# openpsi-project/srl

Hardware: AMD Instinct MI355X
Metric: env-steps/sec through GAE+PPO update, 4096 envs x 128 steps (higher is better)
Workload: dtype f32 (contractions as bf16x3 / f16x2 piece products, float32 accumulate)

## Files before the change

srl_amd/csrc/h2conv.h:

```cpp
#pragma once
#include "h2gemm.h"

namespace srlh2 {

typedef float h2_f32x4 __attribute__((ext_vector_type(4)));

enum { H2C_F2 = 0, H2C_F3 = 1, H2C_D3 = 2, H2C_D2 = 3 };
enum { H2S_LINEAR = 0, H2S_PLANAR = 1, H2S_ROWS = 2, H2S_ROWSWZ = 3 };
enum { H2D_PLANAR = 0, H2D_ROWS = 1, H2D_F32_ROUTED = 2 };

template <int ID> struct H2Geo;

template <> struct H2Geo<H2C_F2> {
  static constexpr int CGW = 1;
  static constexpr int CB = 1, NCH = 64, NTAP = 16, GW = 10, OH = 9, OW = 9, NPIX_L = 400, G = 1, PLANE_E = 400;
  static constexpr int SRC = H2S_ROWSWZ, PAD = 0, SH = 20, SW = 20, SPIX = 400;
  static constexpr int DST = H2D_PLANAR, OPIX = 81, OCH = 64;
  static constexpr bool ZERO_BORDER = false;
  static constexpr bool DENSE = false;
  __host__ __device__ static constexpr int tap_u(int t) { return (((t >> 2) & 1) * 2 + (t & 1)) * 100 + (t >> 3) * 10 + ((t & 3) >> 1); }
  __host__ __device__ static constexpr int tap_k(int t) { return t; }
};
template <> struct H2Geo<H2C_F3> {
  static constexpr int CGW = 1;
  static constexpr int CB = 2, NCH = 64, NTAP = 9, GW = 9, OH = 7, OW = 7, NPIX_L = 81, G = 2, PLANE_E = 176;
  static constexpr int SRC = H2S_PLANAR, PAD = 0, SH = 9, SW = 9, SPIX = 81;
  static constexpr int DST = H2D_ROWS, OPIX = 49, OCH = 64;
  static constexpr bool ZERO_BORDER = false;
  static constexpr bool DENSE = false;
  __host__ __device__ static constexpr int tap_u(int t) { return (t / 3) * 9 + t % 3; }
  __host__ __device__ static constexpr int tap_k(int t) { return t; }
};
template <> struct H2Geo<H2C_D3> {
  static constexpr int CGW = 1;
  static constexpr int CB = 2, NCH = 64, NTAP = 9, GW = 11, OH = 9, OW = 9, NPIX_L = 121, G = 2, PLANE_E = 256;
  static constexpr int SRC = H2S_ROWS, PAD = 2, SH = 7, SW = 7, SPIX = 49;
  static constexpr int DST = H2D_PLANAR, OPIX = 81, OCH = 64;
  static constexpr bool ZERO_BORDER = true;
  static constexpr bool DENSE = true;
  __host__ __device__ static constexpr int tap_u(int t) { return (2 - t / 3) * 11 + (2 - t % 3); }
  __host__ __device__ static constexpr int tap_k(int t) { return t; }
};
template <> struct H2Geo<H2C_D2> {
  static constexpr int CGW = 2;
  static constexpr int CB = 2, NCH = 128, NTAP = 4, GW = 11, OH = 10, OW = 10, NPIX_L = 121, G = 2, PLANE_E = 256;
  static constexpr int SRC = H2S_PLANAR, PAD = 1, SH = 9, SW = 9, SPIX = 81;
  static constexpr int DST = H2D_F32_ROUTED, OPIX = 400, OCH = 32;
  static constexpr bool ZERO_BORDER = true;
  static constexpr bool DENSE = true;
  __host__ __device__ static constexpr int tap_u(int t) { return (1 - t / 2) * 11 + (1 - t % 2); }
  __host__ __device__ static constexpr int tap_k(int t) { return t; }
};

struct H2ConvArgs {
  const void* x;
  const void* w;
  const float* sx;
  const float* sw;
  int64_t n;
  const float* bias;
  int32_t act;
  void* out;
  float* out_scale;
  const float* bound_in;
  const float* bound_w;
  const float* bound_b;
  float* out_absmax;
  uint8_t* mask_out;
  const void* mask_in;
};

#ifdef __HIPCC__

template <int ID> constexpr int h2c_src_img_bytes() { return H2Geo<ID>::SPIX * H2Geo<ID>::CB * 128; }
template <int ID> constexpr int h2c_slot_bytes() { return H2Geo<ID>::CB * 8 * H2Geo<ID>::PLANE_E * 16; }

__device__ __forceinline__ uint32_t h2_xor32(uint32_t x, bool upper) {
#if __has_builtin(__builtin_amdgcn_permlane32_swap)
  typedef unsigned h2_u32x2 __attribute__((ext_vector_type(2)));
  const h2_u32x2 r = __builtin_amdgcn_permlane32_swap(x, x, false, false);
  return upper ? r[0] : r[1];
#else
  (void)upper;
  return (uint32_t)__shfl_xor((int)x, 32);
#endif
}

#ifndef SRL_H2C_SCHED
#define SRL_H2C_SCHED 1
#endif

template <int NKB> struct H2ActiveKb { int n; int kb[NKB]; };
template <int RM, int NTAP, int CB, int TPR> constexpr H2ActiveKb<NTAP * CB> h2_active_kbs() {
  H2ActiveKb<NTAP * CB> a{};
  for (int kb = 0; kb < NTAP * CB; ++kb)
    if ((RM >> ((kb / CB) / TPR)) & 1) a.kb[a.n++] = kb;
  return a;
}

template <int ID, int NSLOT>
__global__ __launch_bounds__(512, 2) void h2conv_kernel(H2ConvArgs a) {
  using GE = H2Geo<ID>;
  constexpr int CB = GE::CB, NKB = GE::NTAP * CB, NPL = CB * 8, PLANE_B = GE::PLANE_E * 16;
  constexpr int SLOT = NPL * PLANE_B;
  constexpr int NCG = GE::NCH / 16;
  constexpr int CGW = GE::CGW, NWG = NCG / CGW;
  constexpr int NPH = 8 / NWG;
  static_assert(NWG == 4 || NWG == 8, "");
  constexpr int NE = GE::DENSE ? GE::OH * GE::OW : (GE::OH - 1) * GE::GW + GE::OW;
  constexpr int NB_IMG = (NE + 15) / 16;
  constexpr int NBT = NB_IMG * GE::G;
  static_assert(NBT % NPH == 0 && NPH <= 2, "blocks split evenly over the (at most two) position halves");
  constexpr int NDMA = SLOT / 1024;
  constexpr int NDW = (NDMA + 7) / 8;
  static_assert(SLOT % 1024 == 0, "");
  constexpr int KROW = NKB * 128;
  constexpr int IMGB = h2c_src_img_bytes<ID>();
  constexpr bool ROUTED = GE::DST == H2D_F32_ROUTED;
  constexpr int OIMGB = GE::OPIX * GE::OCH * 4;
  constexpr int MIMGB = GE::OPIX * GE::OCH / 8;
  constexpr bool MASK_IN = ID == H2C_D3 || ID == H2C_D2, MASK_OUT = !MASK_IN;
  constexpr int MREG = MASK_IN ? (GE::G * MIMGB + 1023) / 1024 * 1024 : 0;
  constexpr int SLOTM = SLOT + MREG;
  constexpr int NDM = MREG / 1024;
  extern __shared__ __attribute__((aligned(1024))) uint8_t lds[];

  const int tid = threadIdx.x, lane = tid & 63;
  const int wid = __builtin_amdgcn_readfirstlane(tid >> 6);
  const int cg0 = (wid % NWG) * CGW, ph = wid / NWG;
  const int p = lane & 15, quad = lane >> 4;
  const bool up = quad >> 1;

  h2_f16x8 wf[CGW][NKB][2];
  {
#pragma unroll
    for (int c = 0; c < CGW; ++c) {
      const uint8_t* wr = static_cast<const uint8_t*>(a.w) + (size_t)((cg0 + c) * 16 + p) * KROW + quad * 32;
#pragma unroll
      for (int kb = 0; kb < NKB; ++kb) {
        wf[c][kb][0] = *reinterpret_cast<const h2_f16x8*>(wr + kb * 128);
        wf[c][kb][1] = *reinterpret_cast<const h2_f16x8*>(wr + kb * 128 + 16);
      }
    }
#pragma unroll
    for (int c = 0; c < CGW; ++c)
#pragma unroll
      for (int kb = 0; kb < NKB; ++kb) asm volatile("" : "+v"(wf[c][kb][0]), "+v"(wf[c][kb][1]));
  }
  const float inv = 1.f / (*a.sx * *a.sw);
  float oscale = 1.f;
  if (!ROUTED) {
    float bound = *a.bound_in * *a.bound_w;
    if (a.bound_b) bound += *a.bound_b;
    oscale = h2_scale_for(bound);
    if (blockIdx.x == 0 && tid == 0) *a.out_scale = oscale;
  }
  float bq[CGW][4];
#pragma unroll
  for (int c = 0; c < CGW; ++c) {
    bq[c][0] = bq[c][1] = bq[c][2] = bq[c][3] = 0.f;
    if (a.bias) {
      const float4 b4 = *reinterpret_cast<const float4*>(a.bias + (cg0 + c) * 16 + 4 * quad);
      bq[c][0] = b4.x; bq[c][1] = b4.y; bq[c][2] = b4.z; bq[c][3] = b4.w;
    }
  }
  const float lo = a.act == 1 ? 0.f : -3.0e38f;

  if (GE::ZERO_BORDER) {
    for (int i = tid; i < NSLOT * SLOTM / 16; i += 512) reinterpret_cast<uint4*>(lds)[i] = make_uint4(0, 0, 0, 0);
    __syncthreads();
  }

  const h2_i32x4 rx = h2_rsrc(a.x);
  h2_i32x4 rmd = h2_rsrc(MASK_IN ? a.mask_in : a.x);
  rmd[2] = MASK_IN ? (int)(a.n * MIMGB) : 0;
  const uint32_t lds0 = (uint32_t)(uintptr_t)(__attribute__((address_space(3))) uint8_t*)lds;
  const long nbatch = (a.n + GE::G - 1) / GE::G;

  uint32_t dvoff[NDW];
  int dimg[NDW];
#pragma unroll
  for (int q = 0; q < NDW; ++q) {
    const int j = wid + 8 * q;
    const int nent = j * 64 + lane;
    if (GE::SRC == H2S_LINEAR) {
      dvoff[q] = (uint32_t)(nent * 16);
      dimg[q] = j < NDMA ? 0 : -1;
    } else if (GE::SRC == H2S_ROWSWZ) {
      const int P = nent >> 3, sl = nent & 7;
      dvoff[q] = (uint32_t)(P * 128 + 16 * (sl ^ (((P >> 1) & 1) | (((P >> 2) & 1) << 2))));
      dimg[q] = j < NDMA ? 0 : -1;
    } else {
      const int plane = nent / GE::PLANE_E, e = nent - plane * GE::PLANE_E;
      const int il = e / GE::NPIX_L, cell = e - il * GE::NPIX_L;
      const int gy = cell / GE::GW, gx = cell - gy * GE::GW;
      const int sy = gy - GE::PAD, sx = gx - GE::PAD;
      const bool ok = j < NDMA && il < GE::G && (unsigned)sy < (unsigned)GE::SH && (unsigned)sx < (unsigned)GE::SW;
      const int sp = sy * GE::SW + sx;
      if (GE::SRC == H2S_PLANAR) dvoff[q] = (uint32_t)(il * IMGB + plane * (GE::SPIX * 16) + sp * 16);
      else dvoff[q] = (uint32_t)((il * GE::SPIX + sp) * (CB * 128) + plane * 16);
      dimg[q] = ok ? il : -1;
      if (!ok) dvoff[q] = 0;
    }
  }
  auto issue = [&](long b, int s) {
    const long img0 = b * GE::G;
    const int left = (int)(a.n - img0 < GE::G ? a.n - img0 : GE::G);
    const uint32_t soff = __builtin_amdgcn_readfirstlane((uint32_t)(img0 * (long)IMGB));
#pragma unroll
    for (int q = 0; q < NDW; ++q) {
      const uint32_t ldsa = __builtin_amdgcn_readfirstlane(lds0 + s * SLOTM + (wid + 8 * q) * 1024);
      if (dimg[q] >= 0 && dimg[q] < left)
        asm volatile("s_mov_b32 m0, %0\n\ts_nop 4\n\tbuffer_load_dwordx4 %1, %2, %3 offen lds" ::"s"(ldsa), "v"(dvoff[q]), "s"(rx), "s"(soff) : "memory");
    }
    if (MASK_IN && wid < NDM) {
      const uint32_t ldsa = __builtin_amdgcn_readfirstlane(lds0 + s * SLOTM + SLOT + wid * 1024);
      const uint32_t msoff = __builtin_amdgcn_readfirstlane((uint32_t)(img0 * (long)MIMGB));
      const uint32_t mvoff = (uint32_t)(wid * 1024 + lane * 16);
      asm volatile("s_mov_b32 m0, %0\n\ts_nop 4\n\tbuffer_load_dwordx4 %1, %2, %3 offen lds" ::"s"(ldsa), "v"(mvoff), "s"(rmd), "s"(msoff) : "memory");
    }
  };

  uint32_t lane_out[CGW];
  uint32_t lane_mout[CGW];
  int mi_shift[CGW], mi_pix[CGW];
  int pix_step_y, pix_step_x;
#pragma unroll
  for (int c = 0; c < CGW; ++c) {
    const int cg = cg0 + c;
    const int g_out = 2 * (quad & 1) + (cg & 1), ocb = cg >> 1;
    if (ROUTED) {
      const int cls = cg >> 1, py = cls >> 1, px = cls & 1;
      lane_out[c] = (uint32_t)(((py * 20 + px) * GE::OCH + 16 * (cg & 1) + 4 * quad) * 4);
      lane_mout[c] = 0;
      mi_shift[c] = 16 * (cg & 1) + 4 * quad;
      mi_pix[c] = py * 20 + px;
    } else {
      lane_out[c] = GE::DST == H2D_PLANAR ? (uint32_t)((((ocb * 4 + g_out) * 2 + (up ? 1 : 0)) * GE::OPIX) * 16)
                                          : (uint32_t)(ocb * 128 + g_out * 32 + (up ? 16 : 0));
      lane_mout[c] = (uint32_t)(ocb * 4 + g_out);
      mi_shift[c] = 0;
      mi_pix[c] = 0;
    }
  }
  if (ROUTED) { pix_step_y = 40; pix_step_x = 2; }
  else { pix_step_y = GE::OW; pix_step_x = 1; }
  constexpr int PIXB = ROUTED ? GE::OCH * 4 : (GE::DST == H2D_PLANAR ? 16 : GE::OCH * 4);
  const uint32_t lane_base = GE::SRC == H2S_ROWSWZ ? (uint32_t)(p * 128 + quad * 32) : (uint32_t)(quad * 2 * PLANE_B + p * 16);
  int swz_d0[8], swz_d1[8];
  if (GE::SRC == H2S_ROWSWZ) {
    static_assert(GE::SRC != H2S_ROWSWZ || SLOTM % 128 == 0, "slot stride must keep address bits 4-6");
    const uint32_t a_ref = (uint32_t)(uintptr_t)(lds + lane_base);
#pragma unroll
    for (int u = 0; u < 8; ++u) {
      const int k = (p + u) & 7;
      const uint32_t x = (uint32_t)((((k >> 1) & 1) | (((k >> 2) & 1) << 2)) * 16);
      swz_d0[u] = u * 128 + (int)((a_ref ^ x) - a_ref);
      swz_d1[u] = u * 128 + (int)((a_ref ^ x ^ 16u) - a_ref);
    }
  }
  float amax = 0.f;

  struct Meta {
    uint32_t pixoff;
    bool ok;
    long img;
    uint32_t bits[CGW];
  };
  const __amdgpu_buffer_rsrc_t r_out = __builtin_amdgcn_make_buffer_rsrc(a.out, 0, (int)(a.n * OIMGB), 0x00020000);
  const __amdgpu_buffer_rsrc_t r_mo = __builtin_amdgcn_make_buffer_rsrc(MASK_OUT ? (void*)a.mask_out : a.out, 0, (int)(a.n * MIMGB), 0x00020000);
  constexpr uint32_t OOB = 0x80000000u;
  auto epilogue1 = [&](const h2_f32x4& acc, const Meta& m, const float (&bqc)[4], uint32_t lane_out_c, uint32_t lane_mout_c, uint32_t mbits) {
    float v[4];
    constexpr bool CLAMP = ID == H2C_F2 || ID == H2C_F3;
#pragma unroll
    for (int r = 0; r < 4; ++r) v[r] = CLAMP ? fmaxf(acc[r] * inv + bqc[r], lo) : acc[r] * inv + bqc[r];
    const bool ok = m.ok;
    const uint32_t img32 = (uint32_t)m.img;
    if (MASK_IN) {
#pragma unroll
      for (int r = 0; r < 4; ++r) v[r] = __uint_as_float(__float_as_uint(v[r]) & (uint32_t)__builtin_amdgcn_sbfe((int)mbits, r, 1));
    }
    {
      const float m3 = __builtin_fmaxf(__builtin_fmaxf(fabsf(v[0]), fabsf(v[1])), fabsf(v[2]));
      const float m5 = __builtin_fmaxf(__builtin_fmaxf(m3, fabsf(v[3])), amax);
      amax = m.ok ? m5 : amax;
    }
    const uint32_t ooff = ok ? m.pixoff * PIXB + lane_out_c : OOB;
    typedef uint32_t h2_u32x4 __attribute__((ext_vector_type(4)));
    if (ROUTED) {
      h2_u32x4 d = {__float_as_uint(v[0]), __float_as_uint(v[1]), __float_as_uint(v[2]), __float_as_uint(v[3])};
      __builtin_amdgcn_raw_buffer_store_b128(d, r_out, ooff + img32 * (uint32_t)OIMGB, 0, 0);
    } else {
      uint32_t h0a, h0b, h1a, h1b;
      h2_split_pair(v[0], v[1], oscale, h0a, h1a);
      h2_split_pair(v[2], v[3], oscale, h0b, h1b);
      h2_u32x4 chunk;
#if __has_builtin(__builtin_amdgcn_permlane32_swap)
      typedef unsigned h2_u32x2 __attribute__((ext_vector_type(2)));
      const h2_u32x2 sa = __builtin_amdgcn_permlane32_swap(h0a, h1a, false, false);
      const h2_u32x2 sb = __builtin_amdgcn_permlane32_swap(h0b, h1b, false, false);
      chunk[0] = sa[0]; chunk[1] = sb[0]; chunk[2] = sa[1]; chunk[3] = sb[1];
#else
      const uint32_t r0 = h2_xor32(up ? h0a : h1a, up), r1 = h2_xor32(up ? h0b : h1b, up);
      chunk[0] = up ? r0 : h0a; chunk[1] = up ? r1 : h0b; chunk[2] = up ? h1a : r0; chunk[3] = up ? h1b : r1;
#endif
      __builtin_amdgcn_raw_buffer_store_b128(chunk, r_out, ooff + img32 * (uint32_t)OIMGB, 0, 0);
      if (MASK_OUT) {
        uint32_t nib = (v[0] > 0.f ? 1u : 0u) | (v[1] > 0.f ? 2u : 0u) | (v[2] > 0.f ? 4u : 0u) | (v[3] > 0.f ? 8u : 0u);
#if __has_builtin(__builtin_amdgcn_permlane32_swap)
        const h2_u32x2 sn = __builtin_amdgcn_permlane32_swap(nib, nib, false, false);
        const uint32_t byte = sn[0] | (sn[1] << 4);
#else
        const uint32_t byte = nib | (h2_xor32(nib, up) << 4);
#endif
        const uint32_t moff = (ok && !up) ? m.pixoff * (GE::OCH / 8) + lane_mout_c : OOB;
        __builtin_amdgcn_raw_buffer_store_b8((unsigned char)byte, r_mo, moff + img32 * (uint32_t)MIMGB, 0, 0);
      }
    }
  };
  auto epilogue = [&](const h2_f32x4 (&accs)[CGW], const Meta& m) {
#pragma unroll
    for (int c = 0; c < CGW; ++c) epilogue1(accs[c], m, bq[c], lane_out[c], lane_mout[c], m.bits[c]);
  };

  constexpr int PD = CB == 1 ? 3 : (ID == H2C_D2 ? 1 : 2);
  const bool late = wid >= 4;
  auto block = [&](auto rows_c, const uint8_t* xb, h2_f32x4 (&pacc)[CGW], Meta& pm, const Meta& nm) {
    constexpr int TPR = ID == H2C_D3 ? 3 : (ID == H2C_D2 ? 2 : GE::NTAP);
    constexpr H2ActiveKb<NKB> AK = h2_active_kbs<decltype(rows_c)::value, GE::NTAP, CB, TPR>();
    h2_f32x4 acc[CGW];
#pragma unroll
    for (int c = 0; c < CGW; ++c) acc[c] = h2_f32x4{0.f, 0.f, 0.f, 0.f};
    h2_f16x8 xr[PD + 1][2];
    const uint8_t* tq0[8];
    const uint8_t* tq1[8];
    if (GE::SRC == H2S_ROWSWZ) {
#pragma unroll
      for (int u = 0; u < 8; ++u) {
        tq0[u] = xb + swz_d0[u];
        tq1[u] = xb + swz_d1[u];
      }
    }
    auto fetch = [&](int i) {
      const int kb = AK.kb[i];
      const int t = kb / CB, c = kb - t * CB;
      if (GE::SRC == H2S_ROWSWZ) {
        const int U = GE::tap_u(t), u8 = U & 7;
        xr[i % (PD + 1)][0] = *reinterpret_cast<const h2_f16x8*>(tq0[u8] + (U - u8) * 128);
        xr[i % (PD + 1)][1] = *reinterpret_cast<const h2_f16x8*>(tq1[u8] + (U - u8) * 128);
      } else {
        const int off = (c * 8) * PLANE_B + GE::tap_u(t) * 16;
        xr[i % (PD + 1)][0] = *reinterpret_cast<const h2_f16x8*>(xb + off);
        xr[i % (PD + 1)][1] = *reinterpret_cast<const h2_f16x8*>(xb + off + PLANE_B);
      }
    };
#pragma unroll
    for (int i = 0; i < PD; ++i) fetch(i);
#pragma unroll
    for (int i = 0; i < AK.n; ++i) {
      if (i + PD < AK.n) fetch(i + PD);
      if (i == 1 && !late) epilogue(pacc, pm);
      if (i == AK.n / 2 + 1 && late) epilogue(pacc, pm);
      const int kb = AK.kb[i];
      const int t = kb / CB, c = kb - t * CB;
      const int kw = GE::tap_k(t) * CB + c;
#pragma unroll
      for (int cc = 0; cc < CGW; ++cc) {
        acc[cc] = __builtin_amdgcn_mfma_f32_16x16x32_f16(wf[cc][kw][1], xr[i % (PD + 1)][0], acc[cc], 0, 0, 0);
        acc[cc] = __builtin_amdgcn_mfma_f32_16x16x32_f16(wf[cc][kw][0], xr[i % (PD + 1)][1], acc[cc], 0, 0, 0);
        acc[cc] = __builtin_amdgcn_mfma_f32_16x16x32_f16(wf[cc][kw][0], xr[i % (PD + 1)][0], acc[cc], 0, 0, 0);
      }
    }
#pragma unroll
    for (int c = 0; c < CGW; ++c) pacc[c] = acc[c];
    pm = nm;
  };

  h2_f32x4 pacc[CGW];
#pragma unroll
  for (int c = 0; c < CGW; ++c) pacc[c] = h2_f32x4{0.f, 0.f, 0.f, 0.f};
  Meta pm = {};
  pm.ok = false;
  auto compute = [&](auto phc_c, long b, int s) {
    constexpr int phc = decltype(phc_c)::value;
    const uint8_t* slot = lds + s * SLOTM + lane_base;
    const uint8_t* mreg = lds + s * SLOTM + SLOT;
#pragma unroll
    for (int jj = 0; jj < NBT / NPH; ++jj) {
      const int jb = phc * (NBT / NPH) + jj;
      const int il = jb / NB_IMG, bi = jb - il * NB_IMG;
      const int e = bi * 16 + p;
      constexpr int EW = GE::DENSE ? GE::OW : GE::GW;
      const int oy = (e * (65536 / EW + 1)) >> 16, ox = e - oy * EW;
      Meta nm;
      nm.img = b * GE::G + il;
      nm.ok = ox < GE::OW && oy < GE::OH && nm.img < a.n;
      nm.pixoff = (uint32_t)(oy * pix_step_y + ox * pix_step_x);
#pragma unroll
      for (int c = 0; c < CGW; ++c) {
        nm.bits[c] = 0u;
        if (MASK_IN) {
          const uint32_t po = nm.ok ? nm.pixoff : 0u;
          if (ID == H2C_D3) nm.bits[c] = (uint32_t)mreg[il * MIMGB + po * (GE::OCH / 8) + lane_mout[c]] >> (up ? 4 : 0);
          else nm.bits[c] = *reinterpret_cast<const uint32_t*>(mreg + il * MIMGB + (po + mi_pix[c]) * 4) >> mi_shift[c];
        }
      }
      const uint8_t* xb_ = slot + (il * GE::NPIX_L + bi * 16) * (GE::SRC == H2S_ROWSWZ ? 128 : 16) +
                           (GE::DENSE ? oy * ((GE::GW - GE::OW) * 16) : 0);
      if (ID == H2C_D3) {
        static_assert(ID != H2C_D3 || (NB_IMG == 6 && GE::GW == 11 && GE::OW == 9 && GE::NTAP == 9 && GE::SRC != H2S_ROWSWZ),
                      "row masks below are conv3's");
        if (bi == 0) block(std::integral_constant<int, 0b011>{}, xb_, pacc, pm, nm);
        else if (bi == 4) block(std::integral_constant<int, 0b110>{}, xb_, pacc, pm, nm);
        else if (bi == 5) block(std::integral_constant<int, 0b100>{}, xb_, pacc, pm, nm);
        else block(std::integral_constant<int, 0b111>{}, xb_, pacc, pm, nm);
      } else if (ID == H2C_D2) {
        static_assert(ID != H2C_D2 || (NB_IMG == 7 && GE::GW == 11 && GE::OW == 10 && GE::NTAP == 4), "row mask below is conv2's");
        if (bi == 6) block(std::integral_constant<int, 0b10>{}, xb_, pacc, pm, nm);
        else block(std::integral_constant<int, 0b11>{}, xb_, pacc, pm, nm);
      } else {
        block(std::integral_constant<int, (1 << 30) - 1>{}, xb_, pacc, pm, nm);
      }
    }
  };

  long b = blockIdx.x;
#pragma unroll
  for (int s = 0; s < NSLOT - 1; ++s)
    if (b + (long)s * gridDim.x < nbatch) issue(b + (long)s * gridDim.x, s);
  int s_cur = 0, s_nxt = NSLOT - 1;
  for (; b < nbatch; b += gridDim.x) {
    asm volatile("s_waitcnt vmcnt(0)\n\ts_waitcnt lgkmcnt(0)" ::: "memory");
    __builtin_amdgcn_s_barrier();
    const long bn = b + (long)(NSLOT - 1) * gridDim.x;
    if (bn < nbatch) issue(bn, s_nxt);
    if (ph == 0) compute(std::integral_constant<int, 0>{}, b, s_cur);
    else compute(std::integral_constant<int, NPH - 1>{}, b, s_cur);
    s_cur = s_cur + 1 == NSLOT ? 0 : s_cur + 1;
    s_nxt = s_nxt + 1 == NSLOT ? 0 : s_nxt + 1;
  }
  epilogue(pacc, pm);
  {
#pragma unroll
    for (int o = 32; o >= 1; o >>= 1) amax = fmaxf(amax, __shfl_xor(amax, o));
    if (lane == 0) {
      const float cur = __hip_atomic_load(a.out_absmax, __ATOMIC_RELAXED, __HIP_MEMORY_SCOPE_AGENT);
      if (amax > cur) atomicMax(reinterpret_cast<int*>(a.out_absmax), __float_as_int(amax));
    }
  }
}

template <int ID, int NSLOT = 2>
inline int h2conv_launch(hipStream_t st, const H2ConvArgs& a, int max_blocks = 256) {
  constexpr bool MASK_IN_L = ID == H2C_D3 || ID == H2C_D2;
  constexpr int SLOT = h2c_slot_bytes<ID>() + (MASK_IN_L ? (H2Geo<ID>::G * (H2Geo<ID>::OPIX * H2Geo<ID>::OCH / 8) + 1023) / 1024 * 1024 : 0);
  static_assert(NSLOT * SLOT <= 160 * 1024, "LDS");
  static bool attr_set = false;
  auto kern = h2conv_kernel<ID, NSLOT>;
  if (!attr_set) {
    (void)hipFuncSetAttribute(reinterpret_cast<const void*>(kern), hipFuncAttributeMaxDynamicSharedMemorySize, NSLOT * SLOT);
    attr_set = true;
  }
  const long nbatch = (a.n + H2Geo<ID>::G - 1) / H2Geo<ID>::G;
  if (nbatch <= 0) return 0;
  const long grid = nbatch < max_blocks ? nbatch : max_blocks;
  hipLaunchKernelGGL(kern, dim3((unsigned)grid), dim3(512), NSLOT * SLOT, st, a);
  return 0;
}

__host__ __device__ inline int h2_entry(int y, int x, int H, int W, int order) {
  return order == 2 ? ((y & 1) * 2 + (x & 1)) * ((H / 2) * (W / 2)) + (y >> 1) * (W / 2) + (x >> 1) : y * W + x;
}
static __global__ void h2_pack_planar_kernel(const float* __restrict__ src, int64_t n, int H, int W, int C, int order, const float* absmax,
                                      const float* scale_in, float* scale_out, uint8_t* __restrict__ dst) {
  const float scale = scale_in ? *scale_in : h2_scale_for(*absmax);
  if (scale_out && blockIdx.x == 0 && threadIdx.x == 0) *scale_out = scale;
  const int64_t ngrp = n * H * W * (C / 8);
  for (int64_t t = (int64_t)blockIdx.x * blockDim.x + threadIdx.x; t < ngrp; t += (int64_t)gridDim.x * blockDim.x) {
    const int gi = (int)(t % (C / 8));
    int64_t r = t / (C / 8);
    const int x = (int)(r % W); r /= W;
    const int y = (int)(r % H);
    const int64_t img = r / H;
    const int blk = gi >> 2, g = gi & 3;
    const float* s = src + ((img * H + y) * W + x) * C + blk * 32;
    float v[8];
#pragma unroll
    for (int j = 0; j < 8; ++j) v[j] = s[h2p_elem(g, j)];
    uint4 h0, h1;
    h2_split_pair(v[0], v[1], scale, h0.x, h1.x);
    h2_split_pair(v[2], v[3], scale, h0.y, h1.y);
    h2_split_pair(v[4], v[5], scale, h0.z, h1.z);
    h2_split_pair(v[6], v[7], scale, h0.w, h1.w);
    const int NP = H * W, e = h2_entry(y, x, H, W, order);
    uint8_t* d = dst + img * (int64_t)(NP * C * 4);
    *reinterpret_cast<uint4*>(d + ((int64_t)((blk * 4 + g) * 2 + 0) * NP + e) * 16) = h0;
    *reinterpret_cast<uint4*>(d + ((int64_t)((blk * 4 + g) * 2 + 1) * NP + e) * 16) = h1;
  }
}
static __global__ void h2_pack_pixrows_kernel(const float* __restrict__ src, int64_t n, int H, int W, int C, int order, const float* absmax,
                                       const float* scale_in, float* scale_out, uint8_t* __restrict__ dst) {
  const float scale = scale_in ? *scale_in : h2_scale_for(*absmax);
  if (scale_out && blockIdx.x == 0 && threadIdx.x == 0) *scale_out = scale;
  const int64_t ngrp = n * H * W * (C / 8);
  for (int64_t t = (int64_t)blockIdx.x * blockDim.x + threadIdx.x; t < ngrp; t += (int64_t)gridDim.x * blockDim.x) {
    const int gi = (int)(t % (C / 8));
    int64_t r = t / (C / 8);
    const int x = (int)(r % W); r /= W;
    const int y = (int)(r % H);
    const int64_t img = r / H;
    const int blk = gi >> 2, g = gi & 3;
    const float* s = src + ((img * H + y) * W + x) * C + blk * 32;
    float v[8];
#pragma unroll
    for (int j = 0; j < 8; ++j) v[j] = s[h2p_elem(g, j)];
    uint4 h0, h1;
    h2_split_pair(v[0], v[1], scale, h0.x, h1.x);
    h2_split_pair(v[2], v[3], scale, h0.y, h1.y);
    h2_split_pair(v[4], v[5], scale, h0.z, h1.z);
    h2_split_pair(v[6], v[7], scale, h0.w, h1.w);
    uint4* d = reinterpret_cast<uint4*>(dst + ((img * (int64_t)(H * W) + h2_entry(y, x, H, W, order)) * C + blk * 32) * 4 + g * 32);
    d[0] = h0;
    d[1] = h1;
  }
}
static __global__ void h2_unpack_planar_kernel(const uint8_t* __restrict__ src, int64_t n, int H, int W, int C, int order, const float* scale,
                                        float* __restrict__ dst) {
  const float inv = 1.f / *scale;
  const int64_t ngrp = n * H * W * (C / 8);
  for (int64_t t = (int64_t)blockIdx.x * blockDim.x + threadIdx.x; t < ngrp; t += (int64_t)gridDim.x * blockDim.x) {
    const int gi = (int)(t % (C / 8));
    int64_t r = t / (C / 8);
    const int x = (int)(r % W); r /= W;
    const int y = (int)(r % H);
    const int64_t img = r / H;
    const int blk = gi >> 2, g = gi & 3;
    const int NP = H * W, e = h2_entry(y, x, H, W, order);
    const uint8_t* d = src + img * (int64_t)(NP * C * 4);
    const _Float16* p0 = reinterpret_cast<const _Float16*>(d + ((int64_t)((blk * 4 + g) * 2 + 0) * NP + e) * 16);
    const _Float16* p1 = reinterpret_cast<const _Float16*>(d + ((int64_t)((blk * 4 + g) * 2 + 1) * NP + e) * 16);
    float* o = dst + ((img * H + y) * W + x) * C + blk * 32;
#pragma unroll
    for (int j = 0; j < 8; ++j) o[h2p_elem(g, j)] = ((float)p0[j] + (float)p1[j]) * inv;
  }
}

#endif

enum { H2W_C2 = 0, H2W_C3 = 1 };

template <int ID> struct H2WGeo;
template <> struct H2WGeo<H2W_C2> {
  static constexpr int CIN = 32, NTAP = 16, GW = 10, OH = 9, OW = 9, XPIX = 400, ZPIX = 81, ZW = 9;
  static constexpr bool X_ROWS = true, Z_ROWS = false;
  static constexpr int MC = 4, NN = 4;
  __host__ __device__ static constexpr int tap_u(int t) { return (((t >> 2) & 1) * 2 + (t & 1)) * 100 + (t >> 3) * 10 + ((t & 3) >> 1); }
};
template <> struct H2WGeo<H2W_C3> {
  static constexpr int CIN = 64, NTAP = 9, GW = 9, OH = 7, OW = 7, XPIX = 81, ZPIX = 49, ZW = 7;
  static constexpr bool X_ROWS = false, Z_ROWS = true;
  static constexpr int MC = 2, NN = 9;
  __host__ __device__ static constexpr int tap_u(int t) { return (t / 3) * 9 + t % 3; }
};

struct H2WgradArgs {
  const void* x;
  const void* dz;
  const float* sx;
  const float* sz;
  int64_t n;
  float* slabs;
};

#ifdef __HIPCC__

typedef short h2_s16x4 __attribute__((ext_vector_type(4)));

__host__ __device__ constexpr int h2w_plane_base(int idx, int plane) { return idx * plane + (idx >> 3) * 256 + (((idx >> 1) & 3) >= 2 ? 128 : 0); }

__device__ __forceinline__ h2_s16x4 h2_tr_read(const uint8_t* p) {
  typedef __attribute__((address_space(3))) h2_s16x4 lds_s16x4;
  return __builtin_amdgcn_ds_read_tr16_b64_v4i16((lds_s16x4*)p);
}

template <int ID, int NSLOT>
__global__ __launch_bounds__(512, 2) void h2wgrad_kernel(H2WgradArgs a) {
  using GE = H2WGeo<ID>;
  constexpr int CBX = GE::CIN / 32;
  constexpr int NE = (GE::OH - 1) * GE::GW + GE::OW;
  constexpr int NCHUNK = (NE + 31) / 32;
  constexpr int ZE = NCHUNK * 32;
  constexpr int ZPLANE = ZE * 16;
  constexpr int ZBYTES = 16 * ZPLANE + 512;
  constexpr int XE = GE::X_ROWS ? GE::XPIX : ((GE::XPIX + 15) / 16) * 16;
  constexpr int XPLANE = XE * 16;
  constexpr int XBYTES = GE::X_ROWS ? GE::XPIX * 128 : CBX * 8 * XPLANE + CBX * 256;
  constexpr int XB_AL = (XBYTES + 1023) / 1024 * 1024, ZB_AL = (ZBYTES + 1023) / 1024 * 1024;
  constexpr int SLOT = XB_AL + ZB_AL;
  constexpr int NDX = XB_AL / 1024, NDZ = ZB_AL / 1024, NDMA = NDX + NDZ, NDW = (NDMA + 7) / 8;
  constexpr int K = GE::NTAP * GE::CIN;
  constexpr int XIMGB = GE::XPIX * GE::CIN * 4, ZIMGB = GE::ZPIX * 64 * 4;
  static_assert(NSLOT * SLOT <= 160 * 1024, "LDS");
  extern __shared__ __attribute__((aligned(1024))) uint8_t lds[];

  const int tid = threadIdx.x, lane = tid & 63;
  const int wid = __builtin_amdgcn_readfirstlane(tid >> 6);
  const int o = lane >> 4, q = (lane >> 2) & 3, p = lane & 3;

  for (int i = tid; i < NSLOT * SLOT / 16; i += 512) reinterpret_cast<uint4*>(lds)[i] = make_uint4(0, 0, 0, 0);
  __syncthreads();

  const h2_i32x4 rx = h2_rsrc(a.x), rz = h2_rsrc(a.dz);
  const uint32_t lds0 = (uint32_t)(uintptr_t)(__attribute__((address_space(3))) uint8_t*)lds;
  int dvoff[NDW];
#pragma unroll
  for (int qd = 0; qd < NDW; ++qd) {
    const int j = wid + 8 * qd;
    int off = -1;
    if (j < NDX) {
      const int b = j * 1024 + lane * 16;
      if (GE::X_ROWS) {
        const int P = b >> 7, sl = (b >> 4) & 7;
        if (P < GE::XPIX) off = P * 128 + 16 * (sl ^ (((P >> 1) & 1) | (((P >> 2) & 1) << 2)));
      } else {
#pragma unroll
        for (int pl_i = 0; pl_i < CBX * 8; ++pl_i) {
          const int rel = b - h2w_plane_base(pl_i, XPLANE);
          if (rel >= 0 && rel < XPLANE && (rel >> 4) < GE::XPIX) off = pl_i * (GE::XPIX * 16) + (rel >> 4) * 16;
        }
      }
    } else if (j < NDMA) {
      const int b = (j - NDX) * 1024 + lane * 16;
#pragma unroll
      for (int pl_i = 0; pl_i < 16; ++pl_i) {
        const int rel = b - h2w_plane_base(pl_i, ZPLANE);
        if (rel >= 0 && rel < ZPLANE) {
          const int e = rel >> 4, oy = e / GE::GW, ox = e - oy * GE::GW;
          if (ox < GE::OW && oy < GE::OH) {
            const int zp = oy * GE::ZW + ox;
            off = GE::Z_ROWS ? zp * 256 + pl_i * 16 : pl_i * (GE::ZPIX * 16) + zp * 16;
          }
        }
      }
    }
    dvoff[qd] = off;
  }
  auto issue = [&](long img, int s) {
    const uint32_t sox = __builtin_amdgcn_readfirstlane((uint32_t)(img * (long)XIMGB));
    const uint32_t soz = __builtin_amdgcn_readfirstlane((uint32_t)(img * (long)ZIMGB));
#pragma unroll
    for (int qd = 0; qd < NDW; ++qd) {
      const int j = wid + 8 * qd;
      const uint32_t ldsa = __builtin_amdgcn_readfirstlane(lds0 + s * SLOT + j * 1024);
      if (dvoff[qd] >= 0) {
        if (j < NDX) asm volatile("s_mov_b32 m0, %0\n\ts_nop 4\n\tbuffer_load_dwordx4 %1, %2, %3 offen lds" ::"s"(ldsa), "v"(dvoff[qd]), "s"(rx), "s"(sox) : "memory");
        else asm volatile("s_mov_b32 m0, %0\n\ts_nop 4\n\tbuffer_load_dwordx4 %1, %2, %3 offen lds" ::"s"(ldsa), "v"(dvoff[qd]), "s"(rz), "s"(soz) : "memory");
      }
    }
  };

  auto zplane = [&](int cb32, int g, int pl) { return h2w_plane_base((cb32 * 4 + g) * 2 + pl, ZPLANE); };
  auto xplane = [&](int cb32, int g, int pl) { return h2w_plane_base((cb32 * 4 + g) * 2 + pl, XPLANE); };
  const int ent = 4 * o + q, half8 = 8 * (p >> 1);
  const int mc0 = GE::MC == 4 ? 0 : (wid & 1) * 2;
  const int nn0 = GE::MC == 4 ? wid * GE::NN : (wid >> 1) * GE::NN;
  uint32_t za[GE::MC];
#pragma unroll
  for (int m = 0; m < GE::MC; ++m) {
    const int cbk = mc0 + m;
    za[m] = (uint32_t)(XB_AL + zplane(cbk >> 1, 2 * (p & 1) + (cbk & 1), 0) + ent * 16 + half8);
  }
  constexpr int CPB = GE::CIN / 16;
  uint32_t swz_lo = 0, swz_hi = 0;
  if (GE::X_ROWS) {
#pragma unroll
    for (int u = 0; u < 8; ++u) {
      const int k = (ent + u) & 7;
      const uint32_t t = (uint32_t)((((k >> 1) & 1) | (((k >> 2) & 1) << 2)) * 16);
      if (u < 4) swz_lo |= t << (8 * u);
      else swz_hi |= t << (8 * (u - 4));
    }
  }

  h2_f32x4 acc[GE::MC][GE::NN];
#pragma unroll
  for (int m = 0; m < GE::MC; ++m)
#pragma unroll
    for (int n2 = 0; n2 < GE::NN; ++n2) acc[m][n2] = h2_f32x4{0.f, 0.f, 0.f, 0.f};
  h2_f32x4 dbacc[2] = {h2_f32x4{0.f, 0.f, 0.f, 0.f}, h2_f32x4{0.f, 0.f, 0.f, 0.f}};
  h2_f16x8 ones;
#pragma unroll
  for (int e = 0; e < 8; ++e) ones[e] = (_Float16)1.0f;

  auto frag = [&](const uint8_t* p0, const uint8_t* p1) {
    union { h2_s16x4 s[2]; h2_f16x8 v; } f;
    f.s[0] = h2_tr_read(p0);
    f.s[1] = h2_tr_read(p1);
    return f.v;
  };
  auto compute = [&](int s) {
    const uint8_t* slot = lds + s * SLOT;
#pragma unroll
    for (int c = 0; c < NCHUNK; ++c) {
      h2_f16x8 af[GE::MC][2];
#pragma unroll
      for (int m = 0; m < GE::MC; ++m)
#pragma unroll
        for (int pl = 0; pl < 2; ++pl) {
          const uint8_t* b = slot + za[m] + pl * ZPLANE + c * 512;
          af[m][pl] = frag(b, b + 256);
        }
      {
        const bool mine = GE::MC == 4 ? wid < 4 : wid < 2;
        if (mine) {
#pragma unroll
          for (int m = 0; m < GE::MC; ++m) {
            if (GE::MC == 4 && m != (wid & 3)) continue;
            h2_f32x4& d = dbacc[GE::MC == 4 ? 0 : (m & 1)];
            d = __builtin_amdgcn_mfma_f32_16x16x32_f16(af[m][0], ones, d, 0, 0, 0);
            d = __builtin_amdgcn_mfma_f32_16x16x32_f16(af[m][1], ones, d, 0, 0, 0);
          }
        }
      }
#pragma unroll
      for (int n2 = 0; n2 < GE::NN; ++n2) {
        const int nn = nn0 + n2;
        const int tap = nn / CPB, c16x = nn - tap * CPB;
        h2_f16x8 xf[2];
        if (GE::X_ROWS) {
          const int U = GE::tap_u(tap);
          const int P0 = c * 32 + U;
          const uint32_t u8 = (uint32_t)(U & 7);
          const uint32_t x = (uint32_t)(((((uint64_t)swz_hi << 32) | swz_lo) >> (8 * u8)) & 0xffu);
          const uint32_t g0 = (uint32_t)((2 * (2 * (p & 1) + c16x)) * 16);
#pragma unroll
          for (int pl = 0; pl < 2; ++pl) {
            const uint32_t a0 = (uint32_t)((P0 + ent) * 128) + ((g0 + pl * 16) ^ x) + half8;
            const uint32_t a1 = (uint32_t)((P0 + ent + 16) * 128) + ((g0 + pl * 16) ^ x) + half8;
            xf[pl] = frag(slot + a0, slot + a1);
          }
        } else {
          const int U = GE::tap_u(tap);
          const int cb32 = c16x >> 1;
#pragma unroll
          for (int pl = 0; pl < 2; ++pl) {
            const uint32_t a0 = (uint32_t)(xplane(cb32, 2 * (p & 1) + (c16x & 1), pl) + (c * 32 + U + ent) * 16 + half8);
            xf[pl] = frag(slot + a0, slot + a0 + 256);
          }
        }
#pragma unroll
        for (int m = 0; m < GE::MC; ++m) {
          acc[m][n2] = __builtin_amdgcn_mfma_f32_16x16x32_f16(af[m][1], xf[0], acc[m][n2], 0, 0, 0);
          acc[m][n2] = __builtin_amdgcn_mfma_f32_16x16x32_f16(af[m][0], xf[1], acc[m][n2], 0, 0, 0);
          acc[m][n2] = __builtin_amdgcn_mfma_f32_16x16x32_f16(af[m][0], xf[0], acc[m][n2], 0, 0, 0);
        }
      }
    }
  };

  long img = blockIdx.x;
#pragma unroll
  for (int s = 0; s < NSLOT - 1; ++s)
    if (img + (long)s * gridDim.x < a.n) issue(img + (long)s * gridDim.x, s);
  int s_cur = 0, s_nxt = NSLOT - 1;
  for (; img < a.n; img += gridDim.x) {
    asm volatile("s_waitcnt vmcnt(0)\n\ts_waitcnt lgkmcnt(0)" ::: "memory");
    __builtin_amdgcn_s_barrier();
    const long in = img + (long)(NSLOT - 1) * gridDim.x;
    if (in < a.n) issue(in, s_nxt);
    compute(s_cur);
    s_cur = s_cur + 1 == NSLOT ? 0 : s_cur + 1;
    s_nxt = s_nxt + 1 == NSLOT ? 0 : s_nxt + 1;
  }

  const float inv = 1.f / (*a.sx * *a.sz);
  float* slab = a.slabs + (size_t)blockIdx.x * (64 * K + 64);
#pragma unroll
  for (int m = 0; m < GE::MC; ++m)
#pragma unroll
    for (int n2 = 0; n2 < GE::NN; ++n2) {
      const int nn = nn0 + n2, tap = nn / CPB, c16x = nn - tap * CPB;
#pragma unroll
      for (int r = 0; r < 4; ++r) {
        const int cout = 16 * (mc0 + m) + 4 * (lane >> 4) + r;
        slab[(size_t)cout * K + tap * GE::CIN + c16x * 16 + (lane & 15)] = acc[m][n2][r] * inv;
      }
    }
  {
    const bool mine = GE::MC == 4 ? wid < 4 : wid < 2;
#pragma unroll
    for (int m = 0; m < (GE::MC == 4 ? 1 : 2); ++m) {
      float t = 0.f;
#pragma unroll
      for (int r = 0; r < 4; ++r) {
        const float v = __shfl(dbacc[m][r], 16 * ((lane & 15) >> 2));
        if ((lane & 3) == r) t = v;
      }
      if (mine && lane < 16) slab[64 * K + 16 * (GE::MC == 4 ? wid : mc0 + m) + lane] = t / *a.sz;
    }
  }
}

static __global__ __launch_bounds__(256) void h2_wgrad_reduce_kernel(const float* __restrict__ slabs, int nslab, int per_slab, int nw,
                                                                     float* __restrict__ gw, float* __restrict__ gb) {
  __shared__ float part[4][64];
  const int o = threadIdx.x & 63, sg = threadIdx.x >> 6;
  const int i = blockIdx.x * 64 + o;
  float s0 = 0.f, s1 = 0.f, s2 = 0.f, s3 = 0.f;
  if (i < per_slab) {
    int k = sg;
    for (; k + 12 < nslab; k += 16) {
      s0 += slabs[(size_t)k * per_slab + i];
      s1 += slabs[(size_t)(k + 4) * per_slab + i];
      s2 += slabs[(size_t)(k + 8) * per_slab + i];
      s3 += slabs[(size_t)(k + 12) * per_slab + i];
    }
    for (; k < nslab; k += 4) s0 += slabs[(size_t)k * per_slab + i];
  }
  part[sg][o] = (s0 + s1) + (s2 + s3);
  __syncthreads();
  if (sg == 0 && i < per_slab) {
    const float s = (part[0][o] + part[1][o]) + (part[2][o] + part[3][o]);
    if (i < nw) gw[i] += s;
    else if (gb) gb[i - nw] += s;
  }
}

template <int ID, int NSLOT>
inline int h2wgrad_launch(hipStream_t st, const H2WgradArgs& a, int grid) {
  using GE = H2WGeo<ID>;
  auto kern = h2wgrad_kernel<ID, NSLOT>;
  constexpr int CBX = GE::CIN / 32;
  constexpr int NE = (GE::OH - 1) * GE::GW + GE::OW, NCHUNK = (NE + 31) / 32, ZE = NCHUNK * 32;
  constexpr int ZBYTES = 16 * ZE * 16 + 512;
  constexpr int XE = GE::X_ROWS ? GE::XPIX : ((GE::XPIX + 15) / 16) * 16;
  constexpr int XBYTES = GE::X_ROWS ? GE::XPIX * 128 : CBX * 8 * XE * 16 + CBX * 256;
  constexpr int SLOT = (XBYTES + 1023) / 1024 * 1024 + (ZBYTES + 1023) / 1024 * 1024;
  static bool attr_set = false;
  if (!attr_set) {
    (void)hipFuncSetAttribute(reinterpret_cast<const void*>(kern), hipFuncAttributeMaxDynamicSharedMemorySize, NSLOT * SLOT);
    attr_set = true;
  }
  hipLaunchKernelGGL(kern, dim3((unsigned)grid), dim3(512), NSLOT * SLOT, st, a);
  return 0;
}

#endif

}
```

Measured before the change: 6.213 million.

## Software-pipeline wgrad conv LDS reads and interleave DMA issue between MFMAs

Restructures the weight-gradient conv kernel's inner loop so each wave group runs a compile-time specialised body: tap and channel indices become constants, X-fragment LDS reads for the next step are double-buffered and issued between MFMAs, and the next Z fragments are prefetched during the last n2 step of each chunk. The DMA issue for the next image is moved from before compute to a fixed point inside the MFMA stream for some wave groups, with sched_barriers pinning the order. The aim is to hide LDS and address-computation latency behind MFMA work and to cut runtime swizzle arithmetic. The cost is code size growing with the eight-way template specialisation, extra register pressure from the double buffers, and a schedule fixed by hand.

After: 6.362 million, median of 6. 2.4% higher.

```diff
diff --git a/srl_amd/csrc/h2conv.h b/srl_amd/csrc/h2conv.h
--- a/srl_amd/csrc/h2conv.h
+++ b/srl_amd/csrc/h2conv.h
@@ -646,25 +646,24 @@
     }
     dvoff[qd] = off;
   }
+  auto issue_one = [&](uint32_t sox, uint32_t soz, int s, int qd) {
+    const int j = wid + 8 * qd;
+    const uint32_t ldsa = __builtin_amdgcn_readfirstlane(lds0 + s * SLOT + j * 1024);
+    if (dvoff[qd] >= 0) {
+      if (j < NDX) asm volatile("s_mov_b32 m0, %0\n\ts_nop 4\n\tbuffer_load_dwordx4 %1, %2, %3 offen lds" ::"s"(ldsa), "v"(dvoff[qd]), "s"(rx), "s"(sox) : "memory");
+      else asm volatile("s_mov_b32 m0, %0\n\ts_nop 4\n\tbuffer_load_dwordx4 %1, %2, %3 offen lds" ::"s"(ldsa), "v"(dvoff[qd]), "s"(rz), "s"(soz) : "memory");
+    }
+  };
   auto issue = [&](long img, int s) {
     const uint32_t sox = __builtin_amdgcn_readfirstlane((uint32_t)(img * (long)XIMGB));
     const uint32_t soz = __builtin_amdgcn_readfirstlane((uint32_t)(img * (long)ZIMGB));
 #pragma unroll
-    for (int qd = 0; qd < NDW; ++qd) {
-      const int j = wid + 8 * qd;
-      const uint32_t ldsa = __builtin_amdgcn_readfirstlane(lds0 + s * SLOT + j * 1024);
-      if (dvoff[qd] >= 0) {
-        if (j < NDX) asm volatile("s_mov_b32 m0, %0\n\ts_nop 4\n\tbuffer_load_dwordx4 %1, %2, %3 offen lds" ::"s"(ldsa), "v"(dvoff[qd]), "s"(rx), "s"(sox) : "memory");
-        else asm volatile("s_mov_b32 m0, %0\n\ts_nop 4\n\tbuffer_load_dwordx4 %1, %2, %3 offen lds" ::"s"(ldsa), "v"(dvoff[qd]), "s"(rz), "s"(soz) : "memory");
-      }
-    }
+    for (int qd = 0; qd < NDW; ++qd) issue_one(sox, soz, s, qd);
   };
 
   auto zplane = [&](int cb32, int g, int pl) { return h2w_plane_base((cb32 * 4 + g) * 2 + pl, ZPLANE); };
-  auto xplane = [&](int cb32, int g, int pl) { return h2w_plane_base((cb32 * 4 + g) * 2 + pl, XPLANE); };
   const int ent = 4 * o + q, half8 = 8 * (p >> 1);
   const int mc0 = GE::MC == 4 ? 0 : (wid & 1) * 2;
-  const int nn0 = GE::MC == 4 ? wid * GE::NN : (wid >> 1) * GE::NN;
   uint32_t za[GE::MC];
 #pragma unroll
   for (int m = 0; m < GE::MC; ++m) {
@@ -672,132 +671,179 @@
     za[m] = (uint32_t)(XB_AL + zplane(cbk >> 1, 2 * (p & 1) + (cbk & 1), 0) + ent * 16 + half8);
   }
   constexpr int CPB = GE::CIN / 16;
-  uint32_t swz_lo = 0, swz_hi = 0;
-  if (GE::X_ROWS) {
-#pragma unroll
-    for (int u = 0; u < 8; ++u) {
-      const int k = (ent + u) & 7;
-      const uint32_t t = (uint32_t)((((k >> 1) & 1) | (((k >> 2) & 1) << 2)) * 16);
-      if (u < 4) swz_lo |= t << (8 * u);
-      else swz_hi |= t << (8 * (u - 4));
-    }
-  }
-
-  h2_f32x4 acc[GE::MC][GE::NN];
-#pragma unroll
-  for (int m = 0; m < GE::MC; ++m)
-#pragma unroll
-    for (int n2 = 0; n2 < GE::NN; ++n2) acc[m][n2] = h2_f32x4{0.f, 0.f, 0.f, 0.f};
-  h2_f32x4 dbacc[2] = {h2_f32x4{0.f, 0.f, 0.f, 0.f}, h2_f32x4{0.f, 0.f, 0.f, 0.f}};
+  constexpr int XG2 = 4 * XPLANE + 128;
+  static_assert(h2w_plane_base(4, XPLANE) - h2w_plane_base(0, XPLANE) == XG2 && h2w_plane_base(7, XPLANE) - h2w_plane_base(3, XPLANE) == XG2 &&
+                    h2w_plane_base(12, XPLANE) - h2w_plane_base(8, XPLANE) == XG2 && h2w_plane_base(15, XPLANE) - h2w_plane_base(11, XPLANE) == XG2,
+                "x planes: lane part");
+  const uint32_t xl_planar = (uint32_t)((p & 1) * XG2 + ent * 16 + half8);
+
   h2_f16x8 ones;
 #pragma unroll
   for (int e = 0; e < 8; ++e) ones[e] = (_Float16)1.0f;
 
-  auto frag = [&](const uint8_t* p0, const uint8_t* p1) {
-    union { h2_s16x4 s[2]; h2_f16x8 v; } f;
-    f.s[0] = h2_tr_read(p0);
-    f.s[1] = h2_tr_read(p1);
-    return f.v;
+  long img = blockIdx.x;
+  const long gstep = gridDim.x;
+#pragma unroll
+  for (int s = 0; s < NSLOT - 1; ++s)
+    if (img + (long)s * gstep < a.n) issue(img + (long)s * gstep, s);
+
+  auto run = [&](auto g_c) {
+    constexpr int G = decltype(g_c)::value;
+    constexpr int nn0 = G * GE::NN;
+    constexpr bool MINE = GE::MC == 4 ? G < 4 : G < 1;
+    constexpr int NP = NCHUNK * GE::NN;
+    uint32_t xl[2][2];
+#pragma unroll
+    for (int t2 = 0; t2 < 2; ++t2)
+#pragma unroll
+      for (int pl = 0; pl < 2; ++pl) {
+        if (GE::X_ROWS) {
+          const int k = (ent + (GE::tap_u(nn0 / CPB + t2) & 7)) & 7;
+          const uint32_t sg = (uint32_t)((((k >> 1) & 1) | (((k >> 2) & 1) << 2)) * 16);
+          xl[t2][pl] = (uint32_t)(ent * 128 + half8) + (((uint32_t)(64 * (p & 1) + 16 * pl)) ^ sg);
+        } else {
+          xl[t2][pl] = xl_planar;
+        }
+      }
+
+    h2_f32x4 acc[GE::MC][GE::NN];
+#pragma unroll
+    for (int m = 0; m < GE::MC; ++m)
+#pragma unroll
+      for (int n2 = 0; n2 < GE::NN; ++n2) acc[m][n2] = h2_f32x4{0.f, 0.f, 0.f, 0.f};
+    h2_f32x4 dbacc[2] = {h2_f32x4{0.f, 0.f, 0.f, 0.f}, h2_f32x4{0.f, 0.f, 0.f, 0.f}};
+
+    union Frag { h2_s16x4 s[2]; h2_f16x8 v; };
+    constexpr int DMA_AT = (GE::MC == 4 ? G >= 4 : G >= 2) ? -1 : 48;
+    static_assert(DMA_AT < NP * 3 * GE::MC, "the DMA block has a gap");
+    auto image = [&](int s, bool dma, long in, int sn) {
+      const uint8_t* slot = lds + s * SLOT;
+      const uint32_t sox = __builtin_amdgcn_readfirstlane((uint32_t)(in * (long)XIMGB));
+      const uint32_t soz = __builtin_amdgcn_readfirstlane((uint32_t)(in * (long)ZIMGB));
+      auto dma_block = [&]() {
+        if (dma) {
+#pragma unroll
+          for (int qd = 0; qd < NDW; ++qd) issue_one(sox, soz, sn, qd);
+        }
+      };
+      if (DMA_AT < 0) dma_block();
+      const uint8_t* zb[GE::MC];
+#pragma unroll
+      for (int m = 0; m < GE::MC; ++m) zb[m] = slot + za[m];
+      const uint8_t* xb[2][2];
+#pragma unroll
+      for (int t2 = 0; t2 < 2; ++t2)
+#pragma unroll
+        for (int pl = 0; pl < 2; ++pl) xb[t2][pl] = slot + xl[t2][pl];
+      Frag af[GE::MC][2], xf[2][2];
+      auto rd_z = [&](int c, int m, int pl, int h) { af[m][pl].s[h] = h2_tr_read(zb[m] + pl * ZPLANE + c * 512 + h * 256); };
+      auto rd_x = [&](int k, int pl, int h) {
+        const int c = k / GE::NN, n2 = k - c * GE::NN;
+        const int nn = nn0 + n2, tap = nn / CPB, c16x = nn - tap * CPB;
+        const int U = GE::tap_u(tap);
+        if constexpr (GE::X_ROWS) xf[k & 1][pl].s[h] = h2_tr_read(xb[tap - nn0 / CPB][pl] + (c * 32 + U + 16 * h) * 128 + 32 * c16x);
+        else xf[k & 1][pl].s[h] = h2_tr_read(xb[0][0] + h2w_plane_base(((c16x >> 1) * 4 + (c16x & 1)) * 2 + pl, XPLANE) + (c * 32 + U) * 16 + h * 256);
+      };
+      rd_x(0, 0, 0); rd_x(0, 0, 1);
+      rd_z(0, 0, 1, 0); rd_z(0, 0, 1, 1);
+      rd_x(0, 1, 0); rd_x(0, 1, 1);
+      rd_z(0, 0, 0, 0); rd_z(0, 0, 0, 1);
+#pragma unroll
+      for (int m = 1; m < GE::MC; ++m) { rd_z(0, m, 1, 0); rd_z(0, m, 1, 1); rd_z(0, m, 0, 0); rd_z(0, m, 0, 1); }
+      __builtin_amdgcn_sched_barrier(0);
+#pragma unroll
+      for (int k = 0; k < NP; ++k) {
+        const int c = k / GE::NN, n2 = k - c * GE::NN, b = k & 1;
+        if (MINE && n2 == 0) {
+#pragma unroll
+          for (int m = 0; m < GE::MC; ++m) {
+            if (GE::MC == 4 && m != (G & 3)) continue;
+            h2_f32x4& d = dbacc[GE::MC == 4 ? 0 : (m & 1)];
+            d = __builtin_amdgcn_mfma_f32_16x16x32_f16(af[m][0].v, ones, d, 0, 0, 0);
+            d = __builtin_amdgcn_mfma_f32_16x16x32_f16(af[m][1].v, ones, d, 0, 0, 0);
+          }
+          __builtin_amdgcn_sched_barrier(0);
+        }
+        const bool more = k + 1 < NP;
+        const bool turn = n2 == GE::NN - 1 && c + 1 < NCHUNK;
+        constexpr int XGAP = GE::MC / 2;
+#pragma unroll
+        for (int m = 0; m < GE::MC; ++m)
+#pragma unroll
+          for (int j = 0; j < 3; ++j) {
+            const int g = 3 * m + j;
+            if (j == 0) acc[m][n2] = __builtin_amdgcn_mfma_f32_16x16x32_f16(af[m][1].v, xf[b][0].v, acc[m][n2], 0, 0, 0);
+            else if (j == 1) acc[m][n2] = __builtin_amdgcn_mfma_f32_16x16x32_f16(af[m][0].v, xf[b][1].v, acc[m][n2], 0, 0, 0);
+            else acc[m][n2] = __builtin_amdgcn_mfma_f32_16x16x32_f16(af[m][0].v, xf[b][0].v, acc[m][n2], 0, 0, 0);
+            if (more && g % XGAP == 0 && g / XGAP < 4) rd_x(k + 1, (g / XGAP) >> 1, (g / XGAP) & 1);
+            if (turn) {
+              if (j == 0) rd_z(c + 1, m, 1, 0);
+              else if (j == 1) rd_z(c + 1, m, 1, 1);
+              else { rd_z(c + 1, m, 0, 0); rd_z(c + 1, m, 0, 1); }
+            }
+            __builtin_amdgcn_sched_barrier(0);
+            if (k * 3 * GE::MC + g == DMA_AT) {
+              dma_block();
+              __builtin_amdgcn_sched_barrier(0);
+            }
+          }
+      }
+    };
+
+    int s_cur = 0, s_nxt = NSLOT - 1;
+    for (; img < a.n; img += gstep) {
+      asm volatile("s_waitcnt vmcnt(0)\n\ts_waitcnt lgkmcnt(0)" ::: "memory");
+      __builtin_amdgcn_s_barrier();
+      const long in = img + (long)(NSLOT - 1) * gstep;
+      image(s_cur, in < a.n, in, s_nxt);
+      s_cur = s_cur + 1 == NSLOT ? 0 : s_cur + 1;
+      s_nxt = s_nxt + 1 == NSLOT ? 0 : s_nxt + 1;
+    }
+
+    const float inv = 1.f / (*a.sx * *a.sz);
+    float* slab = a.slabs + (size_t)blockIdx.x * (64 * K + 64);
+#pragma unroll
+    for (int m = 0; m < GE::MC; ++m)
+#pragma unroll
+      for (int n2 = 0; n2 < GE::NN; ++n2) {
+        const int nn = nn0 + n2, tap = nn / CPB, c16x = nn - tap * CPB;
+#pragma unroll
+        for (int r = 0; r < 4; ++r) {
+          const int cout = 16 * (mc0 + m) + 4 * (lane >> 4) + r;
+          slab[(size_t)cout * K + tap * GE::CIN + c16x * 16 + (lane & 15)] = acc[m][n2][r] * inv;
+        }
+      }
+    if (MINE) {
+#pragma unroll
+      for (int m = 0; m < (GE::MC == 4 ? 1 : 2); ++m) {
+        float t = 0.f;
+#pragma unroll
+        for (int r = 0; r < 4; ++r) {
+          const float v = __shfl(dbacc[m][r], 16 * ((lane & 15) >> 2));
+          if ((lane & 3) == r) t = v;
+        }
+        if (lane < 16) slab[64 * K + 16 * (GE::MC == 4 ? G : mc0 + m) + lane] = t / *a.sz;
+      }
+    }
   };
-  auto compute = [&](int s) {
-    const uint8_t* slot = lds + s * SLOT;
-#pragma unroll
-    for (int c = 0; c < NCHUNK; ++c) {
-      h2_f16x8 af[GE::MC][2];
-#pragma unroll
-      for (int m = 0; m < GE::MC; ++m)
-#pragma unroll
-        for (int pl = 0; pl < 2; ++pl) {
-          const uint8_t* b = slot + za[m] + pl * ZPLANE + c * 512;
-          af[m][pl] = frag(b, b + 256);
-        }
-      {
-        const bool mine = GE::MC == 4 ? wid < 4 : wid < 2;
-        if (mine) {
-#pragma unroll
-          for (int m = 0; m < GE::MC; ++m) {
-            if (GE::MC == 4 && m != (wid & 3)) continue;
-            h2_f32x4& d = dbacc[GE::MC == 4 ? 0 : (m & 1)];
-            d = __builtin_amdgcn_mfma_f32_16x16x32_f16(af[m][0], ones, d, 0, 0, 0);
-            d = __builtin_amdgcn_mfma_f32_16x16x32_f16(af[m][1], ones, d, 0, 0, 0);
-          }
-        }
-      }
-#pragma unroll
-      for (int n2 = 0; n2 < GE::NN; ++n2) {
-        const int nn = nn0 + n2;
-        const int tap = nn / CPB, c16x = nn - tap * CPB;
-        h2_f16x8 xf[2];
-        if (GE::X_ROWS) {
-          const int U = GE::tap_u(tap);
-          const int P0 = c * 32 + U;
-          const uint32_t u8 = (uint32_t)(U & 7);
-          const uint32_t x = (uint32_t)(((((uint64_t)swz_hi << 32) | swz_lo) >> (8 * u8)) & 0xffu);
-          const uint32_t g0 = (uint32_t)((2 * (2 * (p & 1) + c16x)) * 16);
-#pragma unroll
-          for (int pl = 0; pl < 2; ++pl) {
-            const uint32_t a0 = (uint32_t)((P0 + ent) * 128) + ((g0 + pl * 16) ^ x) + half8;
-            const uint32_t a1 = (uint32_t)((P0 + ent + 16) * 128) + ((g0 + pl * 16) ^ x) + half8;
-            xf[pl] = frag(slot + a0, slot + a1);
-          }
-        } else {
-          const int U = GE::tap_u(tap);
-          const int cb32 = c16x >> 1;
-#pragma unroll
-          for (int pl = 0; pl < 2; ++pl) {
-            const uint32_t a0 = (uint32_t)(xplane(cb32, 2 * (p & 1) + (c16x & 1), pl) + (c * 32 + U + ent) * 16 + half8);
-            xf[pl] = frag(slot + a0, slot + a0 + 256);
-          }
-        }
-#pragma unroll
-        for (int m = 0; m < GE::MC; ++m) {
-          acc[m][n2] = __builtin_amdgcn_mfma_f32_16x16x32_f16(af[m][1], xf[0], acc[m][n2], 0, 0, 0);
-          acc[m][n2] = __builtin_amdgcn_mfma_f32_16x16x32_f16(af[m][0], xf[1], acc[m][n2], 0, 0, 0);
-          acc[m][n2] = __builtin_amdgcn_mfma_f32_16x16x32_f16(af[m][0], xf[0], acc[m][n2], 0, 0, 0);
-        }
-      }
-    }
-  };
-
-  long img = blockIdx.x;
-#pragma unroll
-  for (int s = 0; s < NSLOT - 1; ++s)
-    if (img + (long)s * gridDim.x < a.n) issue(img + (long)s * gridDim.x, s);
-  int s_cur = 0, s_nxt = NSLOT - 1;
-  for (; img < a.n; img += gridDim.x) {
-    asm volatile("s_waitcnt vmcnt(0)\n\ts_waitcnt lgkmcnt(0)" ::: "memory");
-    __builtin_amdgcn_s_barrier();
-    const long in = img + (long)(NSLOT - 1) * gridDim.x;
-    if (in < a.n) issue(in, s_nxt);
-    compute(s_cur);
-    s_cur = s_cur + 1 == NSLOT ? 0 : s_cur + 1;
-    s_nxt = s_nxt + 1 == NSLOT ? 0 : s_nxt + 1;
-  }
-
-  const float inv = 1.f / (*a.sx * *a.sz);
-  float* slab = a.slabs + (size_t)blockIdx.x * (64 * K + 64);
-#pragma unroll
-  for (int m = 0; m < GE::MC; ++m)
-#pragma unroll
-    for (int n2 = 0; n2 < GE::NN; ++n2) {
-      const int nn = nn0 + n2, tap = nn / CPB, c16x = nn - tap * CPB;
-#pragma unroll
-      for (int r = 0; r < 4; ++r) {
-        const int cout = 16 * (mc0 + m) + 4 * (lane >> 4) + r;
-        slab[(size_t)cout * K + tap * GE::CIN + c16x * 16 + (lane & 15)] = acc[m][n2][r] * inv;
-      }
-    }
-  {
-    const bool mine = GE::MC == 4 ? wid < 4 : wid < 2;
-#pragma unroll
-    for (int m = 0; m < (GE::MC == 4 ? 1 : 2); ++m) {
-      float t = 0.f;
-#pragma unroll
-      for (int r = 0; r < 4; ++r) {
-        const float v = __shfl(dbacc[m][r], 16 * ((lane & 15) >> 2));
-        if ((lane & 3) == r) t = v;
-      }
-      if (mine && lane < 16) slab[64 * K + 16 * (GE::MC == 4 ? wid : mc0 + m) + lane] = t / *a.sz;
+  const int grp = GE::MC == 4 ? wid : wid >> 1;
+  if (GE::MC == 4) {
+    switch (grp) {
+      case 0: run(std::integral_constant<int, 0>{}); break;
+      case 1: run(std::integral_constant<int, 1>{}); break;
+      case 2: run(std::integral_constant<int, 2>{}); break;
+      case 3: run(std::integral_constant<int, 3>{}); break;
+      case 4: run(std::integral_constant<int, 4>{}); break;
+      case 5: run(std::integral_constant<int, 5>{}); break;
+      case 6: run(std::integral_constant<int, 6>{}); break;
+      default: run(std::integral_constant<int, 7>{}); break;
+    }
+  } else {
+    switch (grp) {
+      case 0: run(std::integral_constant<int, 0>{}); break;
+      case 1: run(std::integral_constant<int, 1>{}); break;
+      case 2: run(std::integral_constant<int, 2>{}); break;
+      default: run(std::integral_constant<int, 3>{}); break;
     }
   }
 }
```
